# ruotianluo/ImageCaptioning.pytorch

Measured on AMD Instinct MI355X. Metric: captions/sec/node (UpDown SCST, bs10xsample_n5, 36x2048 feats), higher is better.
Workload: dtype f32; 1 GPU; UpDown SCST (BASELINE configs[2]): per-GPU batch 10 x train_sample_n 5, 36x2048 bottom-up feats, R=E=1000 A=512, vocab 9487, seq_len 20, references packed+cooked + greedy baseline + CIDEr-D + RewardCriterion + BPTT + clip 0.1 + Adam; rotating_batches=4, global_batch=10, seq_len=20, parallelism=dp1 (flat fp32 gradient, no collective)

## Files before the change

imagecaptioning/pytorch_amd/_lib.py:

```python
import ctypes as C
import os

import torch

HERE = os.path.dirname(os.path.abspath(__file__))
LIB_PATH = os.environ.get('CAPMI_LIB') or os.path.join(HERE, 'libcapmi.so')
MAX_SEG = 4
EINVAL = -1

c_f = C.c_void_p


class GemmSeg(C.Structure):
    _fields_ = [('A', c_f), ('B', c_f), ('lda', C.c_int), ('ldb', C.c_int), ('K', C.c_int), ('a_row_div', C.c_int)]


class GemmDesc(C.Structure):
    _fields_ = [('seg', GemmSeg * MAX_SEG), ('nseg', C.c_int), ('a_layout', C.c_int), ('b_layout', C.c_int),
                ('M', C.c_int), ('N', C.c_int), ('C', c_f), ('ldc', C.c_int), ('bias', c_f), ('bias2', c_f),
                ('row_bias', c_f), ('row_bias_div', C.c_int), ('mul_mask', c_f), ('relu', C.c_int),
                ('accumulate', C.c_int), ('partial', c_f), ('partial_capacity', C.c_int64), ('splits', C.c_int),
                ('defer_reduce', C.c_int), ('splits_used', C.c_int), ('a_planes', c_f * MAX_SEG), ('addend', c_f),
                ('allow_wide_deferred', C.c_int)]


class NextEmbed(C.Structure):
    _fields_ = [('E', c_f), ('mask', c_f), ('x', c_f), ('it_save', c_f), ('Edim', C.c_int), ('relu', C.c_int), ('x_planes', c_f),
                ('alive', c_f)]


class UpDownWeights(C.Structure):
    _fields_ = [(k, c_f) for k in (
        'embed', 'att_w_ih', 'att_w_hh', 'att_b_ih', 'att_b_hh', 'lang_w_ih', 'lang_w_hh', 'lang_b_ih', 'lang_b_hh',
        'h2att_w', 'h2att_b', 'alpha_w', 'alpha_b', 'logit_w', 'logit_b')]


class UpDownRollout(C.Structure):
    _fields_ = ([(k, C.c_int) for k in ('B', 'n', 'N', 'K', 'A', 'R', 'E', 'V1', 'B_feat')] + [('row_img', c_f)] +
                [(k, C.c_int) for k in ('T', 'L')] +
                [(k, c_f) for k in ('fc', 'att', 'p_att', 'att_mask', 'drop_xt', 'drop_out')] +
                [('mode', C.c_int), ('row_mode', c_f), ('temperature', C.c_float), ('gumbel', c_f),
                 ('seed', C.c_uint64), ('forced', c_f), ('forced_ld', C.c_int), ('teacher', C.c_int)] +
                [(k, c_f) for k in ('h_att', 'c_att', 'h_lang', 'c_lang', 'xt', 'it_all', 'gates_att', 'gates_lang',
                                    'att_h', 'alpha', 'ctx', 'h_drop', 'seq', 'seq_logp', 'sel_logp', 'live',
                                    'fc_gates', 'logits', 'it', 'unfinished', 'partial')] +
                [('partial_capacity', C.c_int64), ('top_k', C.c_int), ('top_p', C.c_float), ('ss_mode', c_f),
                 ('planes', c_f), ('planes_bytes', C.c_int64), ('early_exit', C.c_int), ('early_exit_from', C.c_int),
                 ('alive_host', c_f), ('steps_run', C.c_int), ('pre_partial', c_f), ('pre_capacity', C.c_int64), ('raw_logits', C.c_int)])


class SampleFilter(C.Structure):
    _fields_ = [('top_k', C.c_int), ('top_p', C.c_float)]


class UpDownGrads(C.Structure):
    _fields_ = [(k, c_f) for k in (
# ... 322 lines not shown
```

imagecaptioning/pytorch_amd/csrc/gemm_common.h:

```cpp
#pragma once
#include "capmi_common.h"
#include "../../../include/capmi.h"

namespace capmi_gemm {

#ifndef CAPMI_BK
#define CAPMI_BK 32
#endif
constexpr int BK = CAPMI_BK;
constexpr int NT = 256;

struct Seg {
    const float *A, *B;
    int lda, ldb, K, a_row_div;
    int vecA, vecB;
    int rdiv;
    int tstart;
    const unsigned char *Apl;
};

struct KArgs {
    Seg seg[CAPMI_MAX_SEG];
    int nseg;
    int M, N;
    float *C;
    int ldc;
    const float *bias, *bias2, *row_bias;
    int row_bias_div;
    const float *mul_mask;
    int relu, accumulate;
    const float *addend;
    float *partial;
    int splits;
    int to_partial;
    int tiles_total;
    int *counters;
    int self_reduce;
    int sl;
    int ablate;
    int transposed;
};

__device__ __forceinline__ void locate(const KArgs &a, int tile, int &s, int &k0) {
    s = 0;
    int t = tile;
#pragma unroll
    for (int i = 0; i < CAPMI_MAX_SEG; ++i) {
        if (i < a.nseg - 1 && s == i) {
            const int nt = (a.seg[i].K + BK - 1) / BK;
            if (t >= nt) {
                t -= nt;
                s = i + 1;
            }
        }
    }
    k0 = t * BK;
// ... 41 lines not shown
```

imagecaptioning/pytorch_amd/csrc/gemm_f32.hip:

```cpp
#include "host_common.h"
#include "profile.h"
#include "gemm_common.h"
#include <atomic>
#include <stdio.h>
#include <stdlib.h>
#include <hip/hip_ext.h>

using namespace capmi_gemm;

namespace {

template <int ROWS, bool KC>
__device__ __forceinline__ void g2r(f32x4 (&r)[ROWS * BK / 4 / NT], const float *__restrict__ src, int ld,
                                    int row0, int nrows, int k0, int K, int row_div, int vec) {
    constexpr int NV = ROWS * BK / 4 / NT;
#pragma unroll
    for (int p = 0; p < NV; ++p) {
        const int idx = p * NT + threadIdx.x;
        f32x4 v = {0.f, 0.f, 0.f, 0.f};
        if (KC) {
            const int rr = idx / (BK / 4);
            const int kq = (idx % (BK / 4)) * 4;
            const int row = row0 + rr;
            const int k = k0 + kq;
// ... 349 lines not shown
                           bias2, row_bias, row_bias_div > 0 ? row_bias_div : 1, mul_mask, relu, accumulate, ad);
    else
        hipLaunchKernelGGL(splitk_reduce_kernel<false>, dim3(blocks), dim3(256), 0, (hipStream_t)stream, partial, splits, C, ldc, M, N, bias,
                           bias2, row_bias, row_bias_div > 0 ? row_bias_div : 1, mul_mask, relu, accumulate, ad);
    CAPMI_CHECK_LAUNCH();
    return 0;
}

extern "C" int capmi_splitk_reduce(const float *partial, int splits, float *C, int ldc, int M, int N,
                                   const float *bias, const float *bias2, const float *row_bias, int row_bias_div,
                                   const float *mul_mask, int relu, int accumulate, void *stream) {
    return splitk_reduce_addend(partial, splits, C, ldc, M, N, bias, bias2, row_bias, row_bias_div, mul_mask, relu, accumulate, nullptr,
                                stream);
}

extern "C" int capmi_splitk_reduce_batch(const capmi_reduce_item *items, int n_items, void *stream) {
    if (!items || n_items <= 0) return CAPMI_EINVAL;
    hipLaunchKernelGGL(splitk_reduce_batch_kernel, dim3(64, n_items), dim3(256), 0, (hipStream_t)stream, items);
    CAPMI_CHECK_LAUNCH();
    return 0;
}

static std::atomic<int> g_wide_deferred{0};

extern "C" int capmi_gemm_set_policy(int allow_wide_deferred) {
    return g_wide_deferred.exchange(allow_wide_deferred ? 1 : 0);
}

extern "C" int capmi_gemm_f32(capmi_gemm_desc *d, void *stream) {
    if (!d || d->nseg < 1 || d->nseg > CAPMI_MAX_SEG || d->M <= 0 || d->N <= 0 || !d->C) return CAPMI_EINVAL;
    if (d->a_layout < 0 || d->a_layout > 1 || d->b_layout < 0 || d->b_layout > 1) return CAPMI_EINVAL;
    KArgs a{};
    a.nseg = d->nseg;
    int tiles = 0;
    for (int s = 0; s < d->nseg; ++s) {
        const capmi_gemm_seg &g = d->seg[s];
        if (g.K <= 0) return CAPMI_EINVAL;
        if (!g.A || !g.B) return CAPMI_EINVAL;
        Seg &o = a.seg[s];
        o.A = g.A; o.B = g.B; o.lda = g.lda; o.ldb = g.ldb; o.K = g.K;
        o.a_row_div = g.a_row_div > 0 ? g.a_row_div : 1;
        if (d->a_layout == 1 && o.a_row_div != 1) return CAPMI_EINVAL;
        o.vecA = aligned16(g.A) && (g.lda % 4 == 0);
        o.vecB = aligned16(g.B) && (g.ldb % 4 == 0);
        o.rdiv = (65536 + o.a_row_div - 1) / o.a_row_div;
        o.tstart = tiles;
        o.Apl = static_cast<const unsigned char *>(d->a_planes[s]);
        tiles += (g.K + BK - 1) / BK;
    }
    for (int s = d->nseg; s < CAPMI_MAX_SEG; ++s) {
        a.seg[s] = a.seg[0];
        a.seg[s].tstart = 0x7fffffff;
    }
    a.tiles_total = tiles;
    static const int env_ablate = capmi::ablate_env("CAPMI_GEMM_ABLATE");
    a.ablate = env_ablate;
    a.M = d->M; a.N = d->N; a.C = d->C; a.ldc = d->ldc;
    a.bias = d->bias; a.bias2 = d->bias2; a.row_bias = d->row_bias;
    a.row_bias_div = d->row_bias_div > 0 ? d->row_bias_div : 1;
    a.mul_mask = d->mul_mask; a.relu = d->relu; a.accumulate = d->accumulate;
    a.addend = d->addend ? d->addend : d->C;
    const int64_t slab_cap = d->partial ? d->partial_capacity - CAPMI_WS_COUNTER_FLOATS : 0;
    a.partial = d->partial ? d->partial + CAPMI_WS_COUNTER_FLOATS : nullptr;
    a.counters = reinterpret_cast<int *>(d->partial);
    hipStream_t st = (hipStream_t)stream;
    double ksum = 0, abytes = 0;
    for (int s = 0; s < d->nseg; ++s) {
        ksum += d->seg[s].K;
        abytes += (double)d->seg[s].K * ((double)d->M / a.seg[s].a_row_div);
// ... 7 lines not shown
    static const int env_path = capmi::research("CAPMI_GEMM_PATH", 0);
    static const int env_blocks = capmi::research("CAPMI_GEMM_BLOCKS", 512);
    bool ares_ok = d->a_layout == 0 && d->M <= 64 && BK == 32;
    for (int s = 0; s < d->nseg && ares_ok; ++s)
        ares_ok = a.seg[s].vecA && (a.seg[s].K % 4 == 0) && (d->b_layout == 1 || a.seg[s].vecB);
    static const int env_lc = capmi::knob("CAPMI_LC", 1);
    {
        bool lc_ok = env_lc && env_path != 3 && ares_ok && d->M <= 64;
        for (int s = 0; s < d->nseg && lc_ok; ++s)
            lc_ok = d->a_planes[s] != nullptr && a.seg[s].a_row_div == 1 && a.seg[s].vecB;
        if (lc_ok && d->b_layout == 1) lc_ok = d->N % 4 == 0 && d->N >= 4;
        if (lc_ok) {
            static const int env_ab = capmi::research("CAPMI_ARES_BLOCKS", 256);
            static const int env_opt = capmi::research("CAPMI_LC_OPT", 1);
            const int want = d->splits > 0 ? ((d->N + 127) / 128) * d->splits : env_ab;
            int splits = 0;
            a.sl = lc_plan(d->N, tiles, want, &splits);
            const bool partial = splits > 1 || d->defer_reduce;
            if (!partial || (d->partial && (int64_t)splits * d->M * d->N <= slab_cap)) {
                a.splits = splits;
                a.to_partial = partial ? 1 : 0;
                a.self_reduce = 0;
                a.ablate = env_opt;
                d->splits_used = splits;
                int rc = launch_lc(a, d->b_layout, st, pcls, bytes, flops);
                if (rc) return rc;
                if (splits > 1 && !d->defer_reduce)
                    return splitk_reduce_addend(a.partial, splits, d->C, d->ldc, d->M, d->N, d->bias, d->bias2, d->row_bias,
                                               a.row_bias_div, d->mul_mask, d->relu, d->accumulate, d->addend, stream);
                return 0;
            }
        }
    }
    if (env_path != 3 && ares_ok) {
        static const int env_ab = capmi::research("CAPMI_ARES_BLOCKS", 256);
        static const int env_ax3 = capmi::knob("CAPMI_ARES_X3", 1);
        int use_x3 = env_ax3;
        const int want = d->splits > 0 ? ((d->N + 127) / 128) * d->splits : env_ab;
        int splits = 0;
        int ts_cap = ares_ts_cap(d->M, use_x3);
        int ts_max = ares_plan(d->N, tiles, want, ts_cap, &splits);
        if (use_x3 && ((d->N + 127) / 128) * splits > want) {
            const int nblk = (d->N + 127) / 128;
            int splits2 = 0;
            const int ts2 = ares_plan(d->N, tiles, 2 * want, 3, &splits2);
            if (nblk * splits2 <= 2 * want && (int64_t)splits2 * d->M * d->N <= slab_cap) {
                ts_cap = 3; ts_max = ts2; splits = splits2;
            } else {
                int splits32 = 0;
                const int ts32 = ares_plan(d->N, tiles, want, ares_ts_cap(d->M, 0), &splits32);
                if (nblk * splits32 <= want) {
                    use_x3 = 0; ts_cap = ares_ts_cap(d->M, 0); ts_max = ts32; splits = splits32;
                }
            }
        }
        if ((splits > 1 || d->defer_reduce) && (int64_t)splits * d->M * d->N > slab_cap) ts_max = 99;
        if (ts_max <= ts_cap) {
            a.splits = splits;
            a.to_partial = (splits > 1 || d->defer_reduce) ? 1 : 0;
            a.self_reduce = 0;
            static const int env_aopt = capmi::research("CAPMI_ARES_OPT", 2);
            a.ablate = env_aopt;
            if (a.to_partial && (!d->partial || (int64_t)splits * d->M * d->N > slab_cap)) return CAPMI_EINVAL;
            d->splits_used = splits;
            int rc = launch_ares(a, d->b_layout, ts_max, use_x3, st, pcls, bytes, flops);
            if (rc) return rc;
// ... 196 lines not shown
```

imagecaptioning/pytorch_amd/csrc/gemm_lc.hip:

```cpp
#include "gemm_lc_body.h"
#include "profile.h"
#include <hip/hip_ext.h>

namespace capmi_gemm {
namespace {

template <bool BKC, int TM, int ABL = 0, int WAUX = 0>
__global__ __launch_bounds__(LC_NT) void gemm_lc_kernel(const KArgs a) {
    extern __shared__ __attribute__((aligned(16))) unsigned char ldsb[];
    gemm_lc_body<BKC, TM, ABL, WAUX>(a, blockIdx.x, blockIdx.y, gridDim.x, gridDim.y, ldsb);
}

}

int lc_plan(int N, int tiles, int want_blocks, int *splits) {
    const int nblk = (N + LC_BN - 1) / LC_BN;
    int s = want_blocks / nblk;
    if (s < 1) s = 1;
    if (s > tiles) s = tiles;
    int sl = (tiles + s - 1) / s;
    if (sl < 2 && tiles >= 2) sl = 2;
    *splits = (tiles + sl - 1) / sl;
    return sl;
}

template <bool BKC, int TM>
static int launch_lc_t(const KArgs &a, hipStream_t st, int pcls, double bytes, double flops) {
    constexpr size_t lds = (size_t)LC_NS * LC_STAGE;
    static_assert(lds <= 160 * 1024, "ring does not fit the CU's LDS");
    dim3 grid((a.N + LC_BN - 1) / LC_BN, a.splits);
    hipEvent_t e0, e1;
    const bool prof = capmi_prof::take_events(pcls, &e0, &e1, bytes, flops);
    static const int abl = capmi::ablate_env("CAPMI_LC_ABLATE");
#define CAPMI_LC_GO2(A_, W_)                                                                                               \
    do {                                                                                                                   \
        static bool set = false;                                                                                           \
        if (!set) {                                                                                                        \
            (void)hipFuncSetAttribute(reinterpret_cast<const void *>(&gemm_lc_kernel<BKC, TM, A_, W_>),                    \
                                      hipFuncAttributeMaxDynamicSharedMemorySize, 160 * 1024);                             \
            set = true;                                                                                                    \
        }                                                                                                                  \
        if (prof) hipExtLaunchKernelGGL((gemm_lc_kernel<BKC, TM, A_, W_>), grid, dim3(LC_NT), lds, st, e0, e1, 0, a);      \
        else hipLaunchKernelGGL((gemm_lc_kernel<BKC, TM, A_, W_>), grid, dim3(LC_NT), lds, st, a);                         \
    } while (0)
#define CAPMI_LC_GO(A_) CAPMI_LC_GO2(A_, LC_WAUX)
#ifdef CAPMI_VARIANTS
    static const int env_nt = capmi::research("CAPMI_LC_NT", LC_WAUX);
    if (env_nt != LC_WAUX && abl == 0) {
        if (env_nt == 2) CAPMI_LC_GO2(0, 2); else CAPMI_LC_GO2(0, 0);
    } else if constexpr (BKC && TM == 2) {
        switch (abl) {
            case 1: CAPMI_LC_GO(1); break;
            case 2: CAPMI_LC_GO(2); break;
            case 4: CAPMI_LC_GO(4); break;
            case 8: CAPMI_LC_GO(8); break;
            case 3: CAPMI_LC_GO(3); break;
            case 10: CAPMI_LC_GO(10); break;
            case 11: CAPMI_LC_GO(11); break;
            case 15: CAPMI_LC_GO(15); break;
            case 16: CAPMI_LC_GO(16); break;
            case 32: CAPMI_LC_GO(32); break;
            case 64: CAPMI_LC_GO(64); break;
            case 128: CAPMI_LC_GO(128); break;
            case 192: CAPMI_LC_GO(192); break;
            case 160: CAPMI_LC_GO(160); break;
            default: CAPMI_LC_GO(0); break;
        }
    } else {
        CAPMI_LC_GO(0);
    }
#else
    (void)abl;
    CAPMI_LC_GO(0);
#endif
#undef CAPMI_LC_GO
#undef CAPMI_LC_GO2
    CAPMI_CHECK_LAUNCH();
    return 0;
}

thread_local LcCapture *g_lc_capture = nullptr;

int launch_lc(const KArgs &a, int b_layout, hipStream_t st, int pcls, double bytes, double flops) {
    if (a.sl < 1 || a.M > 64 || (long long)a.splits * a.sl < a.tiles_total || (long long)(a.splits - 1) * a.sl >= a.tiles_total)
        return CAPMI_EINVAL;
    if (g_lc_capture) {
        LcCapture &c = *g_lc_capture;
        c.a = a; c.b_layout = b_layout; c.grid_x = (a.N + LC_BN - 1) / LC_BN; c.grid_y = a.splits; c.tm = a.M <= 32 ? 1 : 2;
        c.filled = true;
        return 0;
    }
    if (b_layout == 0) return a.M <= 32 ? launch_lc_t<true, 1>(a, st, pcls, bytes, flops) : launch_lc_t<true, 2>(a, st, pcls, bytes, flops);
    return a.M <= 32 ? launch_lc_t<false, 1>(a, st, pcls, bytes, flops) : launch_lc_t<false, 2>(a, st, pcls, bytes, flops);
}

}
```

imagecaptioning/pytorch_amd/csrc/gemm_lc_body.h:

```cpp
#pragma once
#include "gemm_common.h"

namespace capmi_gemm {
namespace {

constexpr int LC_BN = 128;
constexpr int LC_NT = 768;
constexpr int LC_NS = 5;
constexpr int LC_AB = CAPMI_PL_CHUNK_BYTES;
constexpr int LC_WB = LC_BN * 32 * 4;
constexpr int LC_STAGE = LC_AB + LC_WB;

typedef __bf16 bf16x8 __attribute__((ext_vector_type(8)));
typedef unsigned int u32x4 __attribute__((ext_vector_type(4)));
typedef const void __attribute__((address_space(1))) *gvoid;
typedef void __attribute__((address_space(3))) *lvoid;

constexpr int LC_WAUX = 0;
#define CAPMI_VMCNT(n) __builtin_amdgcn_s_waitcnt((((n) >> 4) << 14) | ((n) & 15) | 0x0f70)

template <bool BKC, int TM, int ABL = 0, int WAUX = 0>
__device__ __forceinline__ void gemm_lc_body(const KArgs &a, const int blk_x, const int blk_y, const int grd_x, const int grd_y,
                                             unsigned char *ldsb) {
    int bx = blk_x, z = blk_y;
    if (a.ablate & 1) {
        const int L = blk_y * grd_x + blk_x, total = grd_x * grd_y;
        const int q = total >> 3, r = total & 7, xcd = L & 7;
        const int p = (xcd < r ? xcd * (q + 1) : r * (q + 1) + (xcd - r) * q) + (L >> 3);
        z = p / grd_x;
        bx = p - z * grd_x;
    }
    const int n0 = bx * LC_BN;
    const int SL = a.sl;
    const int t0 = z * SL;
    const int nst = min(SL, a.tiles_total - t0);
    const int lane = threadIdx.x & 63;
    const int widu = __builtin_amdgcn_readfirstlane((int)(threadIdx.x >> 6));
#define CAPMI_LC_STAMP(slot)                                                                                               \
    do {                                                                                                                   \
        if ((ABL & 16) && lane == 0 && (widu & 7) == 0) {                                                                  \
            __builtin_amdgcn_sched_barrier(0);                                                                             \
            reinterpret_cast<unsigned long long *>(a.counters)[((blk_y * grd_x + blk_x) * 2 + (widu >> 3)) * 10 + (slot)] = \
                __builtin_readcyclecounter();                                                                              \
            __builtin_amdgcn_sched_barrier(0);                                                                             \
        }                                                                                                                  \
    } while (0)
    CAPMI_LC_STAMP(0);

    if (widu >= 8) {
        const int j = widu - 8;
        static_assert(CAPMI_MAX_SEG == 4, "segment selects are written out for 4 segments");
#define CAPMI_PIN(i)                                                                                                       \
        const unsigned char *sgP##i = a.seg[i].Apl; const float *sgB##i = a.seg[i].B;                                      \
        int sgL##i = a.seg[i].ldb, sgK##i = a.seg[i].K, sgT##i = a.seg[i].tstart;                                          \
        asm volatile("" : "+s"(sgP##i), "+s"(sgB##i), "+s"(sgL##i), "+s"(sgK##i), "+s"(sgT##i));
        CAPMI_PIN(0) CAPMI_PIN(1) CAPMI_PIN(2) CAPMI_PIN(3)
#undef CAPMI_PIN
#define CAPMI_SEL(F, tl) ((tl) >= sgT3 ? F##3 : (tl) >= sgT2 ? F##2 : (tl) >= sgT1 ? F##1 : F##0)
        const int N = a.N;
        int wrow[4], wk[4];
#pragma unroll
        for (int u = 0; u < 4; ++u) {
            const int p = j + 4 * u;
            if (BKC) {
                const int cl = 8 * p + (lane >> 3);
                wrow[u] = min(n0 + cl, N - 1);
                wk[u] = 4 * ((lane & 7) ^ ((cl >> 1) & 7));
            } else {
                wrow[u] = 2 * p + (lane >> 5);
                wk[u] = min(n0 + 4 * (lane & 31), N - 4);
            }
        }
        constexpr int DPS = (TM == 2 ? 3 : 2) + 4;
#define CAPMI_LC_ISSUE(i_, slot_idx_)                                                                                      \
        do {                                                                                                               \
            const int tl_ = t0 + (i_);                                                                                     \
            unsigned char *slot_ = ldsb + (slot_idx_) * LC_STAGE;                                                          \
            const int tb_ = CAPMI_SEL(sgT, tl_);                                                                           \
            if (!(ABL & 1)) {                                                                                              \
                const unsigned char *img_ = CAPMI_SEL(sgP, tl_) + (size_t)(tl_ - tb_) * LC_AB + lane * 16;                 \
                _Pragma("unroll") for (int u_ = 0; u_ < (TM == 2 ? 3 : 2); ++u_) {                                         \
                                                                  \
                    int pc_;                                                                                               \
                    if (TM == 2) pc_ = j + 4 * u_;                                                                         \
                    else { const int q_ = min(j + 4 * u_, 5); pc_ = (q_ >> 1) * 4 + (q_ & 1); }                            \
                    __builtin_amdgcn_global_load_lds((gvoid)(uintptr_t)(img_ + pc_ * 1024), (lvoid)(slot_ + pc_ * 1024), 16, 0, 0); \
                }                                                                                                          \
            }                                                                                                              \
            if (!(ABL & 4)) {                                                                                              \
                const int k0_ = (tl_ - tb_) * 32;                                                                          \
                const int ldb_ = CAPMI_SEL(sgL, tl_), brem_ = CAPMI_SEL(sgK, tl_) - k0_;                                   \
                const float *B_ = CAPMI_SEL(sgB, tl_);                                                                     \
// ... 134 lines not shown
            sidx = sidx >= LC_NS - 2 ? sidx + 2 - LC_NS : sidx + 2;
            const bool late = (a.ablate & 2) != 0;
            if (!(ABL & 2)) { wfrag(slot, wb); if (!late) mma(slot, wb, 0); }
            CAPMI_LC_BARRIER();
            ++bars;
            if (!(ABL & 2)) { if (late) mma(slot, wb, 0); mma(slot, wb, 1); }
        }
    }
    while (bars <= nst) { CAPMI_LC_BARRIER(); ++bars; }
    if ((ABL & 128) && blk_x == 0 && blk_y == 0 && lane == 0 && cg == 0)
        printf("lc consumer parity %d: %d ring barriers, %.0f cycles per stage interval, of which %.0f in the barrier\n", par, bars,
               (double)(clock64() - c_t0) / bars, (double)c_bar / bars);
    constexpr int RP = LC_BN + 4;
    float *red = reinterpret_cast<float *>(ldsb);
    CAPMI_LC_BARRIER();
    if (par == 1) {
#pragma unroll
        for (int r = 0; r < 16; ++r) {
            const int row = (r & 3) + 8 * (r >> 2) + 4 * half;
            red[row * RP + cl] = acc0[r];
            if (TM == 2) red[(32 + row) * RP + cl] = acc1[r];
        }
    }
    CAPMI_LC_BARRIER();
#undef CAPMI_LC_BARRIER
    if (par == 1) return;
#pragma unroll
    for (int r = 0; r < 16; ++r) {
        const int row = (r & 3) + 8 * (r >> 2) + 4 * half;
        acc0[r] += red[row * RP + cl];
        if (TM == 2) acc1[r] += red[(32 + row) * RP + cl];
    }
    if (ABL & 16) { asm volatile("" ::"v"(acc0[15]), "v"(acc1[15])); CAPMI_LC_STAMP(2); }
    if ((ABL & 8) || col >= a.N) {
#pragma unroll
        for (int r = 0; r < 16; ++r) { asm volatile("" ::"v"(acc0[r])); asm volatile("" ::"v"(acc1[r])); }
        return;
    }
    if (a.to_partial) {
        float *out = a.partial + (size_t)z * a.M * a.N + col;
#pragma unroll
        for (int r = 0; r < 16; ++r) {
            const int row = (r & 3) + 8 * (r >> 2) + 4 * half;
            if (row < a.M) out[(size_t)row * a.N] = acc0[r];
            if (TM == 2 && row + 32 < a.M) out[(size_t)(row + 32) * a.N] = acc1[r];
        }
        if (ABL & 16) { asm volatile("s_waitcnt vmcnt(0)" ::: "memory"); CAPMI_LC_STAMP(3); }
        return;
    }
    float cb = 0.f;
    if (a.bias) cb += a.bias[col];
    if (a.bias2) cb += a.bias2[col];
#pragma unroll
    for (int i = 0; i < TM; ++i) {
#pragma unroll
        for (int r = 0; r < 16; ++r) {
            const int row = 32 * i + (r & 3) + 8 * (r >> 2) + 4 * half;
            if (row >= a.M) continue;
            float v = (i == 0 ? acc0[r] : acc1[r]) + cb;
            if (a.row_bias) v += a.row_bias[(size_t)(row / a.row_bias_div) * a.N + col];
            if (a.relu) v = fmaxf(v, 0.f);
            if (a.mul_mask) v *= a.mul_mask[(size_t)row * a.N + col];
            if (a.accumulate) v += a.addend[(size_t)row * a.ldc + col];
            a.C[(size_t)row * a.ldc + col] = v;
        }
    }
#undef CAPMI_LC_STAMP
}

}
}
```

imagecaptioning/pytorch_amd/csrc/host_common.h:

```cpp
#pragma once
#include "capmi_common.h"
#include "../../../include/capmi.h"

#define RC(x)                 \
    do {                      \
        int rc__ = (x);       \
        if (rc__) return rc__;\
    } while (0)

#define HIP_RC(x)                                 \
    do {                                          \
        hipError_t e__ = (x);                     \
        if (e__ != hipSuccess) return (int)e__;   \
    } while (0)

inline int grid_for(size_t work, int per_block = 256, int cap = 2048) {
    size_t b = (work + per_block - 1) / per_block;
    if (b > (size_t)cap) b = cap;
    if (b < 1) b = 1;
    return (int)b;
}

template <typename... P>
inline bool aligned16(P... p) {
    return ((... | reinterpret_cast<uintptr_t>(p)) & 15) == 0;
}

struct SegSpec {
    const float *A;
    int lda;
    const float *B;
    int ldb;
    int K;
    int a_row_div;
    const void *Apl;
};

inline int gemm(void *stream, int a_layout, int b_layout, int M, int N, float *C, int ldc, const SegSpec *segs, int nseg,
                float *partial, int64_t cap, int defer, int *splits_used, const float *bias = nullptr,
                const float *bias2 = nullptr, int accumulate = 0, const void *zero_planes = nullptr, int splits_hint = 0) {
    capmi_gemm_desc d{};
    d.nseg = nseg;
    for (int i = 0; i < nseg; ++i) {
        d.seg[i].A = segs[i].A; d.seg[i].lda = segs[i].lda;
        d.seg[i].B = segs[i].B; d.seg[i].ldb = segs[i].ldb;
        d.seg[i].K = segs[i].K; d.seg[i].a_row_div = segs[i].a_row_div > 0 ? segs[i].a_row_div : 1;
        d.a_planes[i] = zero_planes ? segs[i].Apl : nullptr;
    }
    d.a_layout = a_layout; d.b_layout = b_layout;
    d.M = M; d.N = N; d.C = C; d.ldc = ldc;
    d.bias = bias; d.bias2 = bias2;
    d.accumulate = accumulate;
    d.partial = partial; d.partial_capacity = cap;
    d.splits = splits_hint; d.defer_reduce = defer;
    const int rc = capmi_gemm_f32(&d, stream);
    if (splits_used) *splits_used = d.splits_used;
    return rc;
}

inline int dlogits_bwd(bool raw, const capmi_sparse_logp_grad *sparse, const float *g_seq_logp, const float *seq_logp,
                       const uint8_t *live, float *dlogits, int N, int L, int T, int V1, void *stream) {
    if (raw) {
        capmi_sparse_logp_grad sp = sparse ? *sparse : capmi_sparse_logp_grad{};
        sp.raw = 1;
        return capmi_logsoftmax_bwd_sparse(&sp, g_seq_logp, seq_logp, live, dlogits, N, L, T, V1, stream);
    }
    if (sparse) return capmi_logsoftmax_bwd_sparse(sparse, g_seq_logp, seq_logp, live, dlogits, N, L, T, V1, stream);
    return capmi_logsoftmax_bwd(g_seq_logp, seq_logp, live, dlogits, N, L, T, V1, stream);
}
```

imagecaptioning/pytorch_amd/csrc/rollout.hip:

```cpp
#include <chrono>
#include <cstdlib>
#include "host_common.h"

namespace {

inline int64_t pl_chunks(int K) { return (K + 31) / 32; }
constexpr int64_t PL_CHUNK = 12288;

__global__ void tn_to_nt_kernel(const float *__restrict__ src, float *__restrict__ dst, int T, int N, int R) {
    const size_t total = (size_t)T * N * R;
    for (size_t i = (size_t)blockIdx.x * blockDim.x + threadIdx.x; i < total; i += (size_t)gridDim.x * blockDim.x) {
        const int c = (int)(i % R);
        const size_t row = i / R;
        const int n = (int)(row / T), t = (int)(row % T);
        dst[i] = src[((size_t)t * N + n) * R + c];
    }
}

__global__ void pack_recurrent_kernel(const float *__restrict__ lang_ih, const float *__restrict__ lang_hh,
                                      const float *__restrict__ att_ih, const float *__restrict__ att_hh,
                                      float *__restrict__ w_lang_cat, float *__restrict__ w_att_cat, int R, int ld_att_ih) {
    const int R4 = R >> 2;
    const int per_row = 5 * R4;
    const int i = blockIdx.x * blockDim.x + threadIdx.x;
// ... 422 lines not shown
    int n_copies = 0;
    auto colsum = [&](const float *in, int rows, int ncol, float *out, float *out2) -> int {
        for (int i = 0; i < n_grp; ++i)
            if (grp[i].A == in && grp[i].K == rows && grp[i].M == ncol && grp[i].lda == ncol && !grp[i].colsum && n_copies < 4 && aligned16(out)) {
                grp[i].colsum = out;
                if (out2) copies[n_copies++] = Copy2{out2, out, (size_t)ncol * sizeof(float)};
                return 0;
            }
        if (batch_cols) {
            cols[n_cols++] = capmi_colsum_item{in, out, out2, rows, ncol, ncol, 0};
            return 0;
        }
        int rc = capmi_colsum(in, rows, ncol, ncol, out, 0, stream);
        if (rc) return rc;
        if (out2) HIP_RC(hipMemcpyAsync(out2, out, (size_t)ncol * sizeof(float), hipMemcpyDeviceToDevice, (hipStream_t)stream));
        return 0;
    };

    if (phases & CAPMI_BWD_LOGIT) {
        RC(dlogits_bwd(r->raw_logits && !r->teacher, s->sparse, g_seq_logp, r->seq_logp, r->live, s->dlogits, N, L, T, V1, stream));
        SegSpec a{s->dlogits, V1, w->logit_w, R, V1, 1};
        RC(gemm(stream, 0, 1, TN, R, s->d_hdrop, R, &a, 1, P, cap, 0, nullptr));
        SegSpec b{s->dlogits, V1, a_hdrop, R, TN, 1};
        if (side_st) {
            if (hipEventRecord(side_ev[0], st) != hipSuccess) return CAPMI_EINVAL;
            if (hipStreamWaitEvent(side_st, side_ev[0], 0) != hipSuccess) return CAPMI_EINVAL;
            RC(gemm((void *)side_st, 1, 1, V1, R, g->logit_w, R, &b, 1, nullptr, 0, 0, nullptr));
            side_used = true;
        } else if (grouped) grp[n_grp++] = capmi_group_gemm{s->dlogits, a_hdrop, g->logit_w, V1, R, R, TN, V1, R, 0, 0, nullptr};
        else RC(gemm(stream, 1, 1, V1, R, g->logit_w, R, &b, 1, P, cap, 0, nullptr));
        RC(colsum(s->dlogits, TN, V1, g->logit_b, nullptr));
    }

    if (phases & CAPMI_BWD_RECURRENT) {
        const bool al = R % 4 == 0 && ld_att_ih % 4 == 0 &&
                        aligned16(w->lang_w_ih, w->lang_w_hh, w->att_w_ih, w->att_w_hh, s->w_lang_cat, s->w_att_cat);
        if (al) {
            const int total = 4 * R * 5 * R;
            hipLaunchKernelGGL(pack_recurrent_kernel, dim3((total / 4 + 255) / 256), dim3(256), 0, st, w->lang_w_ih, w->lang_w_hh,
                               w->att_w_ih, w->att_w_hh, s->w_lang_cat, s->w_att_cat, R, ld_att_ih);
            CAPMI_CHECK_LAUNCH();
        } else {
            const size_t fb = sizeof(float);
            HIP_RC(hipMemcpy2DAsync(s->w_lang_cat, 3 * R * fb, w->lang_w_ih, 2 * R * fb, 2 * R * fb, 4 * R, hipMemcpyDeviceToDevice, st));
            HIP_RC(hipMemcpy2DAsync(s->w_lang_cat + 2 * R, 3 * R * fb, w->lang_w_hh, R * fb, R * fb, 4 * R, hipMemcpyDeviceToDevice, st));
            HIP_RC(hipMemcpy2DAsync(s->w_att_cat, 2 * R * fb, w->att_w_ih, (size_t)ld_att_ih * fb, R * fb, 4 * R, hipMemcpyDeviceToDevice,
                                    st));
            HIP_RC(hipMemcpy2DAsync(s->w_att_cat + R, 2 * R * fb, w->att_w_hh, R * fb, R * fb, 4 * R, hipMemcpyDeviceToDevice, st));
        }
    }

    const int64_t cap1 = (cap / 4) & ~(int64_t)1023, caph = (cap / 8) & ~(int64_t)1023, capm = cap - cap1 - caph;
    float *P1 = P + capm, *Ph = P + capm + cap1;
    if (phases & CAPMI_BWD_RECURRENT) {
    if (capm <= CAPMI_WS_COUNTER_FLOATS || cap1 <= CAPMI_WS_COUNTER_FLOATS || caph <= CAPMI_WS_COUNTER_FLOATS) return CAPMI_EINVAL;
    static const bool self_reduce = capmi::research("CAPMI_GEMM_SELF_REDUCE", 0) != 0;
    if (self_reduce) {
        HIP_RC(hipMemsetAsync(P1, 0, CAPMI_WS_COUNTER_FLOATS * sizeof(float), st));
        HIP_RC(hipMemsetAsync(Ph, 0, CAPMI_WS_COUNTER_FLOATS * sizeof(float), st));
    }
    unsigned char *pl_dg_lang = nullptr, *pl_dg_att = nullptr, *pl_zero = nullptr;
    if (s->planes && N <= 64 && s->planes_bytes >= capmi_updown_bwd_planes_bytes(R) &&
        (reinterpret_cast<uintptr_t>(s->planes) & 15) == 0) {
        unsigned char *q = static_cast<unsigned char *>(s->planes);
        const int64_t n4 = pl_chunks(4 * R) * PL_CHUNK;
        pl_dg_lang = q; pl_dg_att = q + n4; pl_zero = q + 2 * n4;
    }
    const float *x1_slabs = P1 + CAPMI_WS_COUNTER_FLOATS, *h_slabs = Ph + CAPMI_WS_COUNTER_FLOATS;
    const int64_t x1_stride = (int64_t)N * 2 * R, h_stride = (int64_t)NR;
    int x1_splits = 1, h_splits = 1;
    for (int t = T - 1; t >= 0; --t) {
        const bool last = (t == T - 1);
        float *d_x2 = s->d_x2 + (size_t)t * N * 3 * R;
        const float *d_x2_next = last ? nullptr : s->d_x2 + (size_t)(t + 1) * N * 3 * R;
        float *dg_lang = s->dg_lang + (size_t)t * N * 4 * R;
        float *dg_att = s->dg_att + (size_t)t * N * 4 * R;
        float *dc_lang_in = s->dc_lang + (size_t)((t + 1) & 1) * NR, *dc_lang_out = s->dc_lang + (size_t)(t & 1) * NR;
        float *dc_att_in = s->dc_att + (size_t)((t + 1) & 1) * NR, *dc_att_out = s->dc_att + (size_t)(t & 1) * NR;

        RC(capmi_lstm_cell_bwd_partial_pl(s->d_hdrop + (size_t)t * NR, R, r->drop_out ? r->drop_out + (size_t)t * NRf : nullptr,
                                          last ? nullptr : x1_slabs, 2 * R, x1_splits, x1_stride,
                                          d_x2_next ? d_x2_next + 2 * R : nullptr, 3 * R, 1, 0, last ? nullptr : dc_lang_in,
                                          r->gates_lang + (size_t)t * Nf * 4 * R, r->c_lang + (size_t)t * NRf,
                                          r->c_lang + (size_t)(t + 1) * NRf, dg_lang, dc_lang_out, N, R, pl_dg_lang, stream));
        int x2_splits = 1;
        {
            SegSpec a{dg_lang, 4 * R, s->w_lang_cat, 3 * R, 4 * R, 1, pl_dg_lang};
            RC(gemm(stream, 0, 1, N, 3 * R, P, 3 * R, &a, 1, P, capm, 1, &x2_splits, nullptr, nullptr, 0, pl_zero));
        }
        RC(capmi_attention_bwd_partial(P + CAPMI_WS_COUNTER_FLOATS, x2_splits, (int64_t)N * 3 * R, 3 * R, d_x2,
                                       r->att_h + (size_t)t * Nf * A, r->alpha + (size_t)t * Nf * K, r->p_att, r->att,
                                       w->alpha_w, s->d_att_h_all + (size_t)t * N * A, s->d_e_all + (size_t)t * N * K,
                                       r->B_feat > 0 ? r->B_feat : B, n, K, A, R, r->row_img, N, stream));
        {
            SegSpec a{s->d_att_h_all + (size_t)t * N * A, A, w->h2att_w, R, A, 1};
            RC(gemm(stream, 0, 1, N, R, Ph, R, &a, 1, Ph, caph, 1, &h_splits));
        }
        RC(capmi_lstm_cell_bwd_partial_pl(d_x2 + R, 3 * R, nullptr, h_slabs, R, h_splits, h_stride,
                                          last ? nullptr : x1_slabs + R, 2 * R, x1_splits, x1_stride,
                                          last ? nullptr : dc_att_in, r->gates_att + (size_t)t * Nf * 4 * R,
                                          r->c_att + (size_t)t * NRf, r->c_att + (size_t)(t + 1) * NRf, dg_att, dc_att_out, N, R,
                                          t > 0 ? pl_dg_att : nullptr, stream));
        if (t > 0) {
            SegSpec a{dg_att, 4 * R, s->w_att_cat, 2 * R, 4 * R, 1, pl_dg_att};
            RC(gemm(stream, 0, 1, N, 2 * R, P1, 2 * R, &a, 1, P1, cap1, 1, &x1_splits, nullptr, nullptr, 0, pl_zero));
        }
        if (side_chunks > 1 && t > 0 && t < dw_done_from && chunk_boundary(t)) {
            if (hipEventRecord(side_ev[0], st) != hipSuccess) return CAPMI_EINVAL;
            if (hipStreamWaitEvent(side_st, side_ev[0], 0) != hipSuccess) return CAPMI_EINVAL;
            RC(dw_chunk((void *)side_st, t, dw_done_from, dw_done_from < T ? 1 : 0, nullptr, 0));
            dw_done_from = t;
            side_used = true;
        }
    }

    }

    if (side_used) {
        if (hipEventRecord(side_ev[1], side_st) != hipSuccess) return CAPMI_EINVAL;
        if (hipStreamWaitEvent(st, side_ev[1], 0) != hipSuccess) return CAPMI_EINVAL;
    }
    RC(dw_chunk(stream, 0, dw_done_from, dw_done_from < T ? 1 : 0, P, cap));
    if (phases & CAPMI_BWD_ATT_LSTM) {
        RC(colsum(s->dg_att, TN, 4 * R, g->att_b_ih, g->att_b_hh));
        RC(capmi_group_rowsum(s->dg_att, T, (int64_t)N * 4 * R, B, n, 4 * R, s->sum_dg_att, stream));
        RC(dw_one(stream, 4 * R, R, g->att_w_ih + R, ld_att_ih, s->sum_dg_att, 4 * R, r->fc, R, B, 0, P, cap));
        if (g->d_fc) {
            SegSpec f{s->sum_dg_att, 4 * R, w->att_w_ih + R, ld_att_ih, 4 * R, 1};
            RC(gemm(stream, 0, 1, B, R, g->d_fc, R, &f, 1, P, cap, 0, nullptr));
        }
        SegSpec x{s->dg_att, 4 * R, w->att_w_ih + 2 * R, ld_att_ih, 4 * R, 1};
        RC(gemm(stream, 0, 1, TN, E, s->d_xt_all, E, &x, 1, P, cap, 0, nullptr));
        HIP_RC(hipMemsetAsync(g->embed, 0, (size_t)V1 * E * sizeof(float), st));
        RC(capmi_embed_bwd(a_it, s->d_xt_all, a_xt, a_dropxt, g->embed, TN, E, 1, stream));
    }
    if (phases & CAPMI_BWD_LANG_LSTM) RC(colsum(s->dg_lang, TN, 4 * R, g->lang_b_ih, g->lang_b_hh));
    if (phases & CAPMI_BWD_ATTENTION) {
        RC(colsum(s->d_att_h_all, TN, A, g->h2att_b, nullptr));
// ... 18 lines not shown
```

imagecaptioning/pytorch_amd/ops.py:

```python
import ctypes as C
import os

import torch

from . import _lib
from ._lib import lib, ptr, check, stream_ptr

_f32 = torch.float32


def _chk(*ts):
    for t in ts:
        if t is None:
            continue
        if not t.is_cuda:
            raise _lib.CapmiError('capmi ops need device tensors (got %s)' % t.device)
        if not t.is_contiguous():
            raise _lib.CapmiError('capmi ops need contiguous tensors')


class Workspace:

    COUNTER_FLOATS = 16384

    def __init__(self, device, floats=16 * 1024 * 1024):
        self.buf = torch.zeros(floats + self.COUNTER_FLOATS, dtype=_f32, device=device)

    @property
    def slabs(self):
        return self.buf[self.COUNTER_FLOATS:]

    @property
    def capacity(self):
        return self.buf.numel()


_default_ws = {}


def default_workspace(device):
    key = str(device)
    if key not in _default_ws:
        _default_ws[key] = Workspace(device)
    return _default_ws[key]


def gemm(segs, M, N, out, ldc=None, a_layout=0, b_layout=0, bias=None, bias2=None, row_bias=None, row_bias_div=1,
         mul_mask=None, relu=False, accumulate=False, ws=None, splits=0, defer_reduce=False, a_planes=None, addend=None, stream=None,
         allow_wide=False):
    d = _lib.GemmDesc()
    d.nseg = len(segs)
    if a_planes is not None:
        assert len(a_planes) == len(segs)
        for i, t in enumerate(a_planes):
            d.a_planes[i] = t.data_ptr()
    for i, (A, lda, B, ldb, K, div) in enumerate(segs):
        d.seg[i].A = None if A is None else _addr(A)
        d.seg[i].B = None if B is None else _addr(B)
        d.seg[i].lda, d.seg[i].ldb, d.seg[i].K, d.seg[i].a_row_div = lda, ldb, K, div
    d.a_layout, d.b_layout, d.M, d.N = a_layout, b_layout, M, N
    d.C = _addr(out)
    d.ldc = N if ldc is None else ldc
    d.bias, d.bias2, d.row_bias = ptr(bias), ptr(bias2), ptr(row_bias)
    d.row_bias_div = row_bias_div
    d.mul_mask = ptr(mul_mask)
    d.relu, d.accumulate = int(relu), int(accumulate or addend is not None)
    d.addend = ptr(addend)
    if ws is None:
        ws = default_workspace(_dev(out))
    d.partial, d.partial_capacity = ws.buf.data_ptr(), ws.capacity
    d.splits, d.defer_reduce = splits, int(defer_reduce)
    d.allow_wide_deferred = int(allow_wide)
    check(lib.capmi_gemm_f32(C.byref(d), stream_ptr() if stream is None else stream), 'capmi_gemm_f32')
    return d.splits_used


_zero_planes = {}
_planes_cache = {}


def zero_planes(device, chunks=1):
    key = str(device)
    t = _zero_planes.get(key)
    if t is None or t.numel() < chunks * 12288:
        if torch.cuda.is_current_stream_capturing():
            raise RuntimeError('zero planes requested for the first time inside a graph capture (warm the function up first)')
        t = _zero_planes[key] = torch.zeros(max(chunks, 4) * 12288, dtype=torch.uint8, device=device)
    return t


_capture_scratch = [0]


class capture_scratch:

    def __enter__(self):
        _capture_scratch[0] += 1

    def __exit__(self, *a):
        _capture_scratch[0] -= 1
        return False


def planes_scratch(device, tag, nbytes):
    capturing = torch.cuda.is_current_stream_capturing()
# ... 646 lines not shown
```

include/capmi.h:

```cpp
#ifndef CAPMI_H
#define CAPMI_H

#include <stdint.h>

#ifdef __cplusplus
extern "C" {
#endif

#define CAPMI_EINVAL (-1)
#define CAPMI_MAX_SEG 4
#define CAPMI_WS_COUNTER_FLOATS 16384

int capmi_version(void);
const char *capmi_arch(void);

typedef struct capmi_gemm_seg {
    const float *A;
    const float *B;
    int lda;
    int ldb;
    int K;
    int a_row_div;
} capmi_gemm_seg;

typedef struct capmi_gemm_desc {
    capmi_gemm_seg seg[CAPMI_MAX_SEG];
    int nseg;
    int a_layout;
    int b_layout;
    int M;
    int N;
    float *C;
    int ldc;
    const float *bias;
    const float *bias2;
    const float *row_bias;
    int row_bias_div;
    const float *mul_mask;
    int relu;
    int accumulate;
    float *partial;
    int64_t partial_capacity;
    int splits;
    int defer_reduce;
    int splits_used;
    const void *a_planes[CAPMI_MAX_SEG];
    const float *addend;
    int allow_wide_deferred;
} capmi_gemm_desc;

int capmi_gemm_f32(capmi_gemm_desc *d, void *stream);
int capmi_gemm_set_policy(int allow_wide_deferred);

typedef struct capmi_group_gemm {
    const float *A, *B;
    float *C;
    int32_t lda, ldb, ldc, K, M, N;
    int32_t accumulate;
    int32_t splits_used;
    float *colsum;
} capmi_group_gemm;
int capmi_gemm_group_tn(capmi_group_gemm *items, int n, float *slabs, int64_t slab_floats, void *stream);

int64_t capmi_planes_bytes(int K);
int capmi_planes_from_f32(const float *X, int ld, int M, int K, void *planes, void *stream);

int capmi_attention_fwd(const float *att_h, const float *p_att, const float *att, const float *mask,
                        const float *w, const float *b, float *ctx, float *alpha,
                        int B, int n, int K, int A, int R, const int32_t *row_img, int N, void *stream);

int capmi_attention_fwd_partial(const float *h_partial, int h_splits, int64_t h_stride, const float *h_bias,
                                float *att_h_out, const float *p_att, const float *att, const float *mask,
                                const float *w, const float *b, float *ctx, float *alpha,
                                int B, int n, int K, int A, int R, const int32_t *row_img, int N, void *stream);
int capmi_attention_fwd_partial_pl(const float *h_partial, int h_splits, int64_t h_stride, const float *h_bias,
                                   float *att_h_out, const float *p_att, const float *att, const float *mask,
                                   const float *w, const float *b, float *ctx, float *alpha,
                                   int B, int n, int K, int A, int R, const int32_t *row_img, int N, void *ctx_planes,
                                   void *stream);

int capmi_attention_bwd(const float *d_ctx, int ld_dctx, const float *att_h, const float *alpha,
// ... 646 lines not shown
```

Measured before the change: 12430 captions/s.

## Read recurrent backward weights via column segments instead of packing concatenated copies

Adds column-segment descriptors to the small-M GEMM path, so one GEMM can read its B operand from several separate weight matrices laid side by side in the output columns. The recurrent backward pass uses this to read lang_w_ih/lang_w_hh and att_w_ih/att_w_hh directly, and skips the per-step pack_recurrent_kernel that built concatenated weight copies. The partial-slab store is also rewritten to stage values through LDS and issue 16-byte vector stores. The trade-off is extra per-block segment selection and a new code path that only the LC kernel supports; other paths reject it.

```diff
diff --git a/imagecaptioning/pytorch_amd/_lib.py b/imagecaptioning/pytorch_amd/_lib.py
--- a/imagecaptioning/pytorch_amd/_lib.py
+++ b/imagecaptioning/pytorch_amd/_lib.py
@@ -6,6 +6,7 @@
 HERE = os.path.dirname(os.path.abspath(__file__))
 LIB_PATH = os.environ.get('CAPMI_LIB') or os.path.join(HERE, 'libcapmi.so')
 MAX_SEG = 4
+MAX_BCOL = 3
 EINVAL = -1
 
 c_f = C.c_void_p
@@ -21,7 +22,8 @@
                 ('row_bias', c_f), ('row_bias_div', C.c_int), ('mul_mask', c_f), ('relu', C.c_int),
                 ('accumulate', C.c_int), ('partial', c_f), ('partial_capacity', C.c_int64), ('splits', C.c_int),
                 ('defer_reduce', C.c_int), ('splits_used', C.c_int), ('a_planes', c_f * MAX_SEG), ('addend', c_f),
-                ('allow_wide_deferred', C.c_int)]
+                ('allow_wide_deferred', C.c_int), ('n_bcol', C.c_int), ('bcol_B', c_f * MAX_BCOL), ('bcol_ldb', C.c_int * MAX_BCOL),
+                ('bcol_n', C.c_int * MAX_BCOL)]
 
 
 class NextEmbed(C.Structure):
diff --git a/imagecaptioning/pytorch_amd/csrc/gemm_common.h b/imagecaptioning/pytorch_amd/csrc/gemm_common.h
--- a/imagecaptioning/pytorch_amd/csrc/gemm_common.h
+++ b/imagecaptioning/pytorch_amd/csrc/gemm_common.h
@@ -19,9 +19,17 @@
     const unsigned char *Apl;
 };
 
+constexpr int MAX_BCOL = 3;
+struct BCol {
+    const float *B;
+    int ldb, ncol, blk0, cbase;
+};
+
 struct KArgs {
     Seg seg[CAPMI_MAX_SEG];
     int nseg;
+    int nbcol;
+    BCol bcol[MAX_BCOL];
     int M, N;
     float *C;
     int ldc;
diff --git a/imagecaptioning/pytorch_amd/csrc/gemm_f32.hip b/imagecaptioning/pytorch_amd/csrc/gemm_f32.hip
--- a/imagecaptioning/pytorch_amd/csrc/gemm_f32.hip
+++ b/imagecaptioning/pytorch_amd/csrc/gemm_f32.hip
@@ -405,9 +405,26 @@
     if (d->a_layout < 0 || d->a_layout > 1 || d->b_layout < 0 || d->b_layout > 1) return CAPMI_EINVAL;
     KArgs a{};
     a.nseg = d->nseg;
+    static_assert(CAPMI_MAX_BCOL == MAX_BCOL, "column segments of the descriptor and of the kernel arguments");
+    if (d->n_bcol < 0 || d->n_bcol > MAX_BCOL) return CAPMI_EINVAL;
+    if (d->n_bcol > 0) {
+        if (d->nseg != 1 || d->b_layout != 1) return CAPMI_EINVAL;
+        int ncol = 0, blk = 0;
+        for (int i = 0; i < d->n_bcol; ++i) {
+            if (!d->bcol_B[i] || d->bcol_n[i] <= 0 || d->bcol_n[i] % 4 || d->bcol_ldb[i] % 4 || d->bcol_ldb[i] < d->bcol_n[i] ||
+                !aligned16(d->bcol_B[i]))
+                return CAPMI_EINVAL;
+            a.bcol[i] = BCol{d->bcol_B[i], d->bcol_ldb[i], d->bcol_n[i], blk, ncol};
+            ncol += d->bcol_n[i];
+            blk += (d->bcol_n[i] + 127) / 128;
+        }
+        if (ncol != d->N) return CAPMI_EINVAL;
+        a.nbcol = d->n_bcol;
+    }
     int tiles = 0;
     for (int s = 0; s < d->nseg; ++s) {
-        const capmi_gemm_seg &g = d->seg[s];
+        capmi_gemm_seg g = d->seg[s];
+        if (a.nbcol) { g.B = a.bcol[0].B; g.ldb = a.bcol[0].ldb; }
         if (g.K <= 0) return CAPMI_EINVAL;
         if (!g.A || !g.B) return CAPMI_EINVAL;
         Seg &o = a.seg[s];
@@ -481,6 +498,7 @@
             }
         }
     }
+    if (a.nbcol) return CAPMI_EINVAL;
     if (env_path != 3 && ares_ok) {
         static const int env_ab = capmi::research("CAPMI_ARES_BLOCKS", 256);
         static const int env_ax3 = capmi::knob("CAPMI_ARES_X3", 1);
diff --git a/imagecaptioning/pytorch_amd/csrc/gemm_lc.hip b/imagecaptioning/pytorch_amd/csrc/gemm_lc.hip
--- a/imagecaptioning/pytorch_amd/csrc/gemm_lc.hip
+++ b/imagecaptioning/pytorch_amd/csrc/gemm_lc.hip
@@ -24,11 +24,16 @@
     return sl;
 }
 
+static int lc_grid_x(const KArgs &a) {
+    if (a.nbcol <= 0) return (a.N + LC_BN - 1) / LC_BN;
+    return a.bcol[a.nbcol - 1].blk0 + (a.bcol[a.nbcol - 1].ncol + LC_BN - 1) / LC_BN;
+}
+
 template <bool BKC, int TM>
 static int launch_lc_t(const KArgs &a, hipStream_t st, int pcls, double bytes, double flops) {
     constexpr size_t lds = (size_t)LC_NS * LC_STAGE;
     static_assert(lds <= 160 * 1024, "ring does not fit the CU's LDS");
-    dim3 grid((a.N + LC_BN - 1) / LC_BN, a.splits);
+    dim3 grid(lc_grid_x(a), a.splits);
     hipEvent_t e0, e1;
     const bool prof = capmi_prof::take_events(pcls, &e0, &e1, bytes, flops);
     static const int abl = capmi::ablate_env("CAPMI_LC_ABLATE");
@@ -84,9 +89,10 @@
 int launch_lc(const KArgs &a, int b_layout, hipStream_t st, int pcls, double bytes, double flops) {
     if (a.sl < 1 || a.M > 64 || (long long)a.splits * a.sl < a.tiles_total || (long long)(a.splits - 1) * a.sl >= a.tiles_total)
         return CAPMI_EINVAL;
+    if (a.nbcol < 0 || a.nbcol > MAX_BCOL || (a.nbcol > 0 && (b_layout != 1 || a.nseg != 1))) return CAPMI_EINVAL;
     if (g_lc_capture) {
         LcCapture &c = *g_lc_capture;
-        c.a = a; c.b_layout = b_layout; c.grid_x = (a.N + LC_BN - 1) / LC_BN; c.grid_y = a.splits; c.tm = a.M <= 32 ? 1 : 2;
+        c.a = a; c.b_layout = b_layout; c.grid_x = lc_grid_x(a); c.grid_y = a.splits; c.tm = a.M <= 32 ? 1 : 2;
         c.filled = true;
         return 0;
     }
diff --git a/imagecaptioning/pytorch_amd/csrc/gemm_lc_body.h b/imagecaptioning/pytorch_amd/csrc/gemm_lc_body.h
--- a/imagecaptioning/pytorch_amd/csrc/gemm_lc_body.h
+++ b/imagecaptioning/pytorch_amd/csrc/gemm_lc_body.h
@@ -30,7 +30,19 @@
         z = p / grd_x;
         bx = p - z * grd_x;
     }
-    const int n0 = bx * LC_BN;
+    int n0 = bx * LC_BN, ncols = a.N, obase = 0;
+    const float *cB = nullptr;
+    int cL = 0;
+    if (!BKC && a.nbcol > 0) {
+        static_assert(MAX_BCOL == 3, "column-segment selects are written out for 3 segments");
+        const int j = (a.nbcol > 2 && bx >= a.bcol[2].blk0) ? 2 : (a.nbcol > 1 && bx >= a.bcol[1].blk0) ? 1 : 0;
+        const int b0 = j == 2 ? a.bcol[2].blk0 : j == 1 ? a.bcol[1].blk0 : 0;
+        n0 = (bx - b0) * LC_BN;
+        ncols = j == 2 ? a.bcol[2].ncol : j == 1 ? a.bcol[1].ncol : a.bcol[0].ncol;
+        obase = j == 2 ? a.bcol[2].cbase : j == 1 ? a.bcol[1].cbase : a.bcol[0].cbase;
+        cB = j == 2 ? a.bcol[2].B : j == 1 ? a.bcol[1].B : a.bcol[0].B;
+        cL = j == 2 ? a.bcol[2].ldb : j == 1 ? a.bcol[1].ldb : a.bcol[0].ldb;
+    }
     const int SL = a.sl;
     const int t0 = z * SL;
     const int nst = min(SL, a.tiles_total - t0);
@@ -56,8 +68,12 @@
         asm volatile("" : "+s"(sgP##i), "+s"(sgB##i), "+s"(sgL##i), "+s"(sgK##i), "+s"(sgT##i));
         CAPMI_PIN(0) CAPMI_PIN(1) CAPMI_PIN(2) CAPMI_PIN(3)
 #undef CAPMI_PIN
+        if (!BKC && cB) {
+            sgB0 = cB; sgL0 = cL;
+            asm volatile("" : "+s"(sgB0), "+s"(sgL0));
+        }
 #define CAPMI_SEL(F, tl) ((tl) >= sgT3 ? F##3 : (tl) >= sgT2 ? F##2 : (tl) >= sgT1 ? F##1 : F##0)
-        const int N = a.N;
+        const int N = ncols;
         int wrow[4], wk[4];
 #pragma unroll
         for (int u = 0; u < 4; ++u) {
@@ -258,25 +274,51 @@
         if (TM == 2) acc1[r] += red[(32 + row) * RP + cl];
     }
     if (ABL & 16) { asm volatile("" ::"v"(acc0[15]), "v"(acc1[15])); CAPMI_LC_STAMP(2); }
-    if ((ABL & 8) || col >= a.N) {
+    if (ABL & 8) {
 #pragma unroll
         for (int r = 0; r < 16; ++r) { asm volatile("" ::"v"(acc0[r])); asm volatile("" ::"v"(acc1[r])); }
         return;
     }
     if (a.to_partial) {
-        float *out = a.partial + (size_t)z * a.M * a.N + col;
-#pragma unroll
-        for (int r = 0; r < 16; ++r) {
-            const int row = (r & 3) + 8 * (r >> 2) + 4 * half;
-            if (row < a.M) out[(size_t)row * a.N] = acc0[r];
-            if (TM == 2 && row + 32 < a.M) out[(size_t)(row + 32) * a.N] = acc1[r];
+        float *slab = a.partial + (size_t)z * a.M * a.N + obase;
+        const int ldo = a.N;
+        const bool v16 = ((ldo | obase | ncols) & 3) == 0 && (reinterpret_cast<uintptr_t>(a.partial) & 15) == 0;
+        if (v16) {
+#pragma unroll
+            for (int r = 0; r < 16; ++r) {
+                const int row = (r & 3) + 8 * (r >> 2) + 4 * half;
+                red[row * RP + cl] = acc0[r];
+                if (TM == 2) red[(32 + row) * RP + cl] = acc1[r];
+            }
+            asm volatile("s_waitcnt lgkmcnt(0)" ::: "memory");
+            __builtin_amdgcn_wave_barrier();
+            const int pc = n0 + 32 * cg + 4 * (lane & 7);
+            if (pc < ncols) {
+#pragma unroll
+                for (int it = 0; it < 8 * TM; ++it) {
+                    const int row = 8 * it + (lane >> 3);
+                    const f32x4 v = *reinterpret_cast<const f32x4 *>(red + row * RP + 32 * cg + 4 * (lane & 7));
+                    float *dst = slab + (size_t)row * ldo + pc;
+                    if (row < a.M) asm volatile("global_store_dwordx4 %0, %1, off sc1\n\ts_nop 1" ::"v"(dst), "v"(v) : "memory");
+                }
+            }
+        } else if (col < ncols) {
+#pragma unroll
+            for (int r = 0; r < 16; ++r) {
+                const int row = (r & 3) + 8 * (r >> 2) + 4 * half;
+                if (row < a.M) __hip_atomic_store(slab + (size_t)row * ldo + col, acc0[r], __ATOMIC_RELAXED, __HIP_MEMORY_SCOPE_AGENT);
+                if (TM == 2 && row + 32 < a.M)
+                    __hip_atomic_store(slab + (size_t)(row + 32) * ldo + col, acc1[r], __ATOMIC_RELAXED, __HIP_MEMORY_SCOPE_AGENT);
+            }
         }
         if (ABL & 16) { asm volatile("s_waitcnt vmcnt(0)" ::: "memory"); CAPMI_LC_STAMP(3); }
         return;
     }
+    if (col >= ncols) return;
+    const int oc = obase + col;
     float cb = 0.f;
-    if (a.bias) cb += a.bias[col];
-    if (a.bias2) cb += a.bias2[col];
+    if (a.bias) cb += a.bias[oc];
+    if (a.bias2) cb += a.bias2[oc];
 #pragma unroll
     for (int i = 0; i < TM; ++i) {
 #pragma unroll
@@ -284,11 +326,11 @@
             const int row = 32 * i + (r & 3) + 8 * (r >> 2) + 4 * half;
             if (row >= a.M) continue;
             float v = (i == 0 ? acc0[r] : acc1[r]) + cb;
-            if (a.row_bias) v += a.row_bias[(size_t)(row / a.row_bias_div) * a.N + col];
+            if (a.row_bias) v += a.row_bias[(size_t)(row / a.row_bias_div) * a.N + oc];
             if (a.relu) v = fmaxf(v, 0.f);
-            if (a.mul_mask) v *= a.mul_mask[(size_t)row * a.N + col];
-            if (a.accumulate) v += a.addend[(size_t)row * a.ldc + col];
-            a.C[(size_t)row * a.ldc + col] = v;
+            if (a.mul_mask) v *= a.mul_mask[(size_t)row * a.N + oc];
+            if (a.accumulate) v += a.addend[(size_t)row * a.ldc + oc];
+            a.C[(size_t)row * a.ldc + oc] = v;
         }
     }
 #undef CAPMI_LC_STAMP
diff --git a/imagecaptioning/pytorch_amd/csrc/host_common.h b/imagecaptioning/pytorch_amd/csrc/host_common.h
--- a/imagecaptioning/pytorch_amd/csrc/host_common.h
+++ b/imagecaptioning/pytorch_amd/csrc/host_common.h
@@ -36,9 +36,15 @@
     const void *Apl;
 };
 
+struct BColSpec {
+    const float *B;
+    int ldb, ncol;
+};
+
 inline int gemm(void *stream, int a_layout, int b_layout, int M, int N, float *C, int ldc, const SegSpec *segs, int nseg,
                 float *partial, int64_t cap, int defer, int *splits_used, const float *bias = nullptr,
-                const float *bias2 = nullptr, int accumulate = 0, const void *zero_planes = nullptr, int splits_hint = 0) {
+                const float *bias2 = nullptr, int accumulate = 0, const void *zero_planes = nullptr, int splits_hint = 0,
+                const BColSpec *bcols = nullptr, int nbcol = 0) {
     capmi_gemm_desc d{};
     d.nseg = nseg;
     for (int i = 0; i < nseg; ++i) {
@@ -53,6 +59,8 @@
     d.accumulate = accumulate;
     d.partial = partial; d.partial_capacity = cap;
     d.splits = splits_hint; d.defer_reduce = defer;
+    d.n_bcol = nbcol;
+    for (int i = 0; i < nbcol && i < CAPMI_MAX_BCOL; ++i) { d.bcol_B[i] = bcols[i].B; d.bcol_ldb[i] = bcols[i].ldb; d.bcol_n[i] = bcols[i].ncol; }
     const int rc = capmi_gemm_f32(&d, stream);
     if (splits_used) *splits_used = d.splits_used;
     return rc;
diff --git a/imagecaptioning/pytorch_amd/csrc/rollout.hip b/imagecaptioning/pytorch_amd/csrc/rollout.hip
--- a/imagecaptioning/pytorch_amd/csrc/rollout.hip
+++ b/imagecaptioning/pytorch_amd/csrc/rollout.hip
@@ -478,9 +478,16 @@
         RC(colsum(s->dlogits, TN, V1, g->logit_b, nullptr));
     }
 
-    if (phases & CAPMI_BWD_RECURRENT) {
-        const bool al = R % 4 == 0 && ld_att_ih % 4 == 0 &&
-                        aligned16(w->lang_w_ih, w->lang_w_hh, w->att_w_ih, w->att_w_hh, s->w_lang_cat, s->w_att_cat);
+    const int64_t cap1 = (cap / 4) & ~(int64_t)1023, caph = (cap / 8) & ~(int64_t)1023, capm = cap - cap1 - caph;
+    float *P1 = P + capm, *Ph = P + capm + cap1;
+    static const int env_pack = capmi::knob("CAPMI_BWD_PACK", 0);
+    static const int env_lc = capmi::knob("CAPMI_LC", 1);
+    const bool w_al = R % 4 == 0 && ld_att_ih % 4 == 0 && aligned16(w->lang_w_ih, w->lang_w_hh, w->att_w_ih, w->att_w_hh);
+    const bool colseg = !env_pack && env_lc && w_al && N <= 64 && s->planes && s->planes_bytes >= capmi_updown_bwd_planes_bytes(R) &&
+                        (reinterpret_cast<uintptr_t>(s->planes) & 15) == 0 && aligned16(s->dg_lang, s->dg_att) &&
+                        (cap1 < capm ? cap1 : capm) - CAPMI_WS_COUNTER_FLOATS >= (int64_t)N * 256 * 128;
+    if ((phases & CAPMI_BWD_RECURRENT) && !colseg) {
+        const bool al = w_al && aligned16(s->w_lang_cat, s->w_att_cat);
         if (al) {
             const int total = 4 * R * 5 * R;
             hipLaunchKernelGGL(pack_recurrent_kernel, dim3((total / 4 + 255) / 256), dim3(256), 0, st, w->lang_w_ih, w->lang_w_hh,
@@ -496,8 +503,6 @@
         }
     }
 
-    const int64_t cap1 = (cap / 4) & ~(int64_t)1023, caph = (cap / 8) & ~(int64_t)1023, capm = cap - cap1 - caph;
-    float *P1 = P + capm, *Ph = P + capm + cap1;
     if (phases & CAPMI_BWD_RECURRENT) {
     if (capm <= CAPMI_WS_COUNTER_FLOATS || cap1 <= CAPMI_WS_COUNTER_FLOATS || caph <= CAPMI_WS_COUNTER_FLOATS) return CAPMI_EINVAL;
     static const bool self_reduce = capmi::research("CAPMI_GEMM_SELF_REDUCE", 0) != 0;
@@ -532,7 +537,8 @@
         int x2_splits = 1;
         {
             SegSpec a{dg_lang, 4 * R, s->w_lang_cat, 3 * R, 4 * R, 1, pl_dg_lang};
-            RC(gemm(stream, 0, 1, N, 3 * R, P, 3 * R, &a, 1, P, capm, 1, &x2_splits, nullptr, nullptr, 0, pl_zero));
+            const BColSpec bc[2] = {{w->lang_w_ih, 2 * R, 2 * R}, {w->lang_w_hh, R, R}};
+            RC(gemm(stream, 0, 1, N, 3 * R, P, 3 * R, &a, 1, P, capm, 1, &x2_splits, nullptr, nullptr, 0, pl_zero, 0, bc, colseg ? 2 : 0));
         }
         RC(capmi_attention_bwd_partial(P + CAPMI_WS_COUNTER_FLOATS, x2_splits, (int64_t)N * 3 * R, 3 * R, d_x2,
                                        r->att_h + (size_t)t * Nf * A, r->alpha + (size_t)t * Nf * K, r->p_att, r->att,
@@ -549,7 +555,8 @@
                                           t > 0 ? pl_dg_att : nullptr, stream));
         if (t > 0) {
             SegSpec a{dg_att, 4 * R, s->w_att_cat, 2 * R, 4 * R, 1, pl_dg_att};
-            RC(gemm(stream, 0, 1, N, 2 * R, P1, 2 * R, &a, 1, P1, cap1, 1, &x1_splits, nullptr, nullptr, 0, pl_zero));
+            const BColSpec bc[2] = {{w->att_w_ih, ld_att_ih, R}, {w->att_w_hh, R, R}};
+            RC(gemm(stream, 0, 1, N, 2 * R, P1, 2 * R, &a, 1, P1, cap1, 1, &x1_splits, nullptr, nullptr, 0, pl_zero, 0, bc, colseg ? 2 : 0));
         }
         if (side_chunks > 1 && t > 0 && t < dw_done_from && chunk_boundary(t)) {
             if (hipEventRecord(side_ev[0], st) != hipSuccess) return CAPMI_EINVAL;
diff --git a/imagecaptioning/pytorch_amd/ops.py b/imagecaptioning/pytorch_amd/ops.py
--- a/imagecaptioning/pytorch_amd/ops.py
+++ b/imagecaptioning/pytorch_amd/ops.py
@@ -47,7 +47,7 @@
 
 def gemm(segs, M, N, out, ldc=None, a_layout=0, b_layout=0, bias=None, bias2=None, row_bias=None, row_bias_div=1,
          mul_mask=None, relu=False, accumulate=False, ws=None, splits=0, defer_reduce=False, a_planes=None, addend=None, stream=None,
-         allow_wide=False):
+         allow_wide=False, b_cols=None):
     d = _lib.GemmDesc()
     d.nseg = len(segs)
     if a_planes is not None:
@@ -71,6 +71,10 @@
     d.partial, d.partial_capacity = ws.buf.data_ptr(), ws.capacity
     d.splits, d.defer_reduce = splits, int(defer_reduce)
     d.allow_wide_deferred = int(allow_wide)
+    if b_cols:
+        d.n_bcol = len(b_cols)
+        for i, (B, ldb, ncol) in enumerate(b_cols):
+            d.bcol_B[i], d.bcol_ldb[i], d.bcol_n[i] = _addr(B), ldb, ncol
     check(lib.capmi_gemm_f32(C.byref(d), stream_ptr() if stream is None else stream), 'capmi_gemm_f32')
     return d.splits_used
 
diff --git a/include/capmi.h b/include/capmi.h
--- a/include/capmi.h
+++ b/include/capmi.h
@@ -9,6 +9,7 @@
 
 #define CAPMI_EINVAL (-1)
 #define CAPMI_MAX_SEG 4
+#define CAPMI_MAX_BCOL 3
 #define CAPMI_WS_COUNTER_FLOATS 16384
 
 int capmi_version(void);
@@ -47,6 +48,10 @@
     const void *a_planes[CAPMI_MAX_SEG];
     const float *addend;
     int allow_wide_deferred;
+    int n_bcol;
+    const float *bcol_B[CAPMI_MAX_BCOL];
+    int bcol_ldb[CAPMI_MAX_BCOL];
+    int bcol_n[CAPMI_MAX_BCOL];
 } capmi_gemm_desc;
 
 int capmi_gemm_f32(capmi_gemm_desc *d, void *stream);
```

Result: faster. 12630 captions/s (median of 6 runs) (+1.6%).
